# OpenPPL/ppl.llm.serving

Hardware: AMD Instinct MI355X
Metric: decode tokens/sec, LLaMA-7B int8 (W8A16), max-running-batch 1024 (higher is better)
Workload: dtype fp16 activations, int8 weights (W8A16), int8-g8 KV, fp32 accumulate

## Files before the change

### include/pplhip.h

```cpp
#ifndef PPLHIP_H_
#define PPLHIP_H_

#include <stdint.h>
#include <stddef.h>

#ifdef __cplusplus
extern "C" {
#endif

#define PPLHIP_API __attribute__((visibility("default")))

typedef enum pplhip_status {
    PPLHIP_SUCCESS = 0,
    PPLHIP_OTHER_ERROR = -1,
    PPLHIP_INVALID_VALUE = -2,
    PPLHIP_OUT_OF_MEMORY = -3,
    PPLHIP_DEVICE_RUNTIME_ERROR = -4,
    PPLHIP_DEVICE_MEMORY_ERROR = -5,
    PPLHIP_NOT_FOUND = -6,
    PPLHIP_UNSUPPORTED = -7
} pplhip_status;

typedef struct pplhip_model_desc {
    int32_t hidden_dim;
// ... 208 lines not shown
    void* cache;
    void* scale;
    int64_t max_tokens;
    int32_t num_layers;
    int32_t kv_heads;
    int32_t head_dim;
    int32_t quant_bit, quant_group, layout, mode, page_size;
    int32_t layer;
} pplhip_kv_view;

PPLHIP_API int pplhip_op_rope_kv_write(void* stream, void* qkv, const float* cos_sin, const pplhip_kv_view* kv,
                                       const int64_t* seq_starts, const int64_t* start_pos,
                                       const int64_t* cache_indices, int64_t max_pages, int64_t B, int64_t T,
                                       int32_t num_heads);

PPLHIP_API int pplhip_op_attention(void* stream, const void* qkv, const pplhip_kv_view* kv,
                                   const int64_t* seq_starts, const int64_t* start_pos,
                                   const int64_t* cache_indices, int64_t max_pages, int64_t B, int64_t T,
                                   int64_t decoding_batches, int64_t max_seq_len, int64_t max_kv_len,
                                   int32_t num_heads, int32_t split_k, void* workspace, uint64_t workspace_bytes,
                                   void* out);

PPLHIP_API int pplhip_build_rope_table(float* host_out, int32_t max_position, int32_t head_dim, float theta);

#ifdef __cplusplus
}
#endif

#endif
```

### ppl.llm.serving_amd/csrc/k_gemm_dev.h

```cpp
#pragma once
#include "kernels.h"
#include "k_launch.h"

namespace pplhip {

constexpr int G_BN = 128, G_BM = 128, G_BK = 64;

__device__ __forceinline__ int g_swz(int row, int chunk) { return chunk ^ ((row >> 1) & 7); }

enum { EPI_F16 = 0, EPI_F32 = 1, EPI_SWIGLU = 2 };
template <int EPI>
__device__ __forceinline__ void store4(void* yv, int64_t ldy, int64_t m, int n, float v0, float v1, float v2, float v3) {
    if constexpr (EPI == EPI_F32) {
        *reinterpret_cast<float4*>(reinterpret_cast<float*>(yv) + m * ldy + n) = make_float4(v0, v1, v2, v3);
    } else if constexpr (EPI == EPI_F16) {
        const h4 o = {to_h(v0), to_h(v1), to_h(v2), to_h(v3)};
        *reinterpret_cast<uint2*>(reinterpret_cast<uint16_t*>(yv) + m * ldy + n) = __builtin_bit_cast(uint2, o);
    } else {
        const float g0 = round_h(v0), u0 = round_h(v1), g1 = round_h(v2), u1 = round_h(v3);
        const h2 o = {to_h(g0 / (1.0f + __expf(-g0)) * u0), to_h(g1 / (1.0f + __expf(-g1)) * u1)};
        *reinterpret_cast<uint32_t*>(reinterpret_cast<uint16_t*>(yv) + m * ldy + (n >> 1)) = __builtin_bit_cast(uint32_t, o);
    }
}

template <class F>
// ... 288 lines not shown
```

### ppl.llm.serving_amd/csrc/k_gemm_wide.hip

```cpp
#include <stdlib.h>
#include "k_gemm_dev.h"

namespace pplhip {

namespace {

constexpr int WD_BM = 128, WD_NP = 4;
constexpr int WD_XB = WD_BM * G_BK * 2;
constexpr int WD_XP = WD_XB / 1024;

template <int EPI, int ST, int NC, int ABL = 0>
__global__ __launch_bounds__((NC + WD_NP) * 64) void gemm_w8_wide_kernel(const uint16_t* __restrict__ x, const int8_t* __restrict__ w,
                                                                  const uint16_t* __restrict__ scale, int64_t M, int N, int K,
                                                                  void* __restrict__ yv, int64_t ldy, int n_tiles, int m_tiles) {
    constexpr int WD_BN = 32 * NC, WD_NC = NC;
    constexpr int WD_WB = WD_BN * G_BK, WD_WP = WD_WB / 1024;
    constexpr int WD_PP = (WD_XP + WD_WP + WD_NP - 1) / WD_NP;
    extern __shared__ __attribute__((aligned(16))) char smem_wd[];
    char* const Xs0 = smem_wd;
    char* const Wq0 = smem_wd + ST * WD_XB;

    const int id = blockIdx.x;
    const int xcd = id & 7, slot = id >> 3;
    const int nt = xcd + 8 * (slot / m_tiles);
    const int mt = slot % m_tiles;
    if (nt >= n_tiles) return;
    const int n0 = nt * WD_BN;
    const int64_t m0 = (int64_t)mt * WD_BM;

// ... 40 lines not shown
            const int younger = (ktiles - 1 - t) < (D - 1) ? (ktiles - 1 - t) : (D - 1);
            if (younger >= 2) {
                if (npc == WD_PP) asm volatile("s_waitcnt vmcnt(%0)" ::"n"(2 * WD_PP) : "memory");
                else asm volatile("s_waitcnt vmcnt(%0)" ::"n"(2 * WD_PP - 2) : "memory");
            } else if (younger == 1) {
                if (npc == WD_PP) asm volatile("s_waitcnt vmcnt(%0)" ::"n"(WD_PP) : "memory");
                else asm volatile("s_waitcnt vmcnt(%0)" ::"n"(WD_PP - 1) : "memory");
            } else {
                asm volatile("s_waitcnt vmcnt(0)" ::: "memory");
            }
            if (!(ABL & 8)) __syncthreads();
            if (t + D < ktiles && !(ABL & 1)) WD_PRODUCE(t + D, stn);
            stn = stn == ST - 1 ? 0 : stn + 1;
        }
#undef WD_PRODUCE
        return;
    }

    const int l15 = lane & 15, kq = lane >> 4;
    const int nb = wave * 32;
    f4 acc[2][8];
#pragma unroll
    for (int i = 0; i < 2; ++i)
#pragma unroll
        for (int j = 0; j < 8; ++j) acc[i][j] = f4{0.f, 0.f, 0.f, 0.f};
    int st = 0;
    for (int t = 0; t < ktiles; ++t) {
        if (!(ABL & 8)) __syncthreads();
        const uint16_t* xs = reinterpret_cast<const uint16_t*>(Xs0 + st * WD_XB);
        const char* wq = Wq0 + st * WD_WB;
// ... 12 lines not shown
                if constexpr (ABL & 2) a[i] = __builtin_bit_cast(h8, make_uint4(wraw[i].x, wraw[i].y, wraw[i].z ^ ks, wraw[i].w));
                else a[i] = cvt_i8x8_f16(ks == 0 ? make_uint2(wraw[i].x, wraw[i].y) : make_uint2(wraw[i].z, wraw[i].w));
            }
#pragma unroll
            for (int j = 0; j < 8; ++j) {
                const int row = j * 16 + l15;
                bfr[j] = __builtin_bit_cast(h8, *reinterpret_cast<const uint4*>(&xs[((ABL & 4) ? 0 : row * G_BK) + g_swz(row, ks * 4 + kq) * 8]));
            }
#pragma unroll
            for (int i = 0; i < 2; ++i)
#pragma unroll
                for (int j = 0; j < 8; ++j) acc[i][j] = __builtin_amdgcn_mfma_f32_16x16x32_f16(a[i], bfr[j], acc[i][j], 0, 0, 0);
        }
    }

#pragma unroll
    for (int i = 0; i < 2; ++i) {
        const int n = n0 + nb + i * 16 + kq * 4;
        if (n >= N) continue;
        const h4 sh = __builtin_bit_cast(h4, *reinterpret_cast<const uint2*>(scale + n));
#pragma unroll
        for (int j = 0; j < 8; ++j) {
            const int64_t m = m0 + j * 16 + l15;
            if (m >= M) continue;
            store4<EPI>(yv, ldy, m, n, acc[i][j][0] * (float)sh[0], acc[i][j][1] * (float)sh[1], acc[i][j][2] * (float)sh[2],
                        acc[i][j][3] * (float)sh[3]);
        }
    }
}

// ... 15 lines not shown
    const size_t lds = (size_t)ST * (WD_XB + bn * G_BK);
    if (route) {
        route->add("kernel=gemm_w8_wide_kernel<%s,%d,%d> splits=1 reduce=none order=plain", epi_name(epi), ST, nc);
        if (route->dry) return hipSuccess;
    }
    static LdsOptIn once;
    if (once.first()) set_max_lds(lds, gemm_w8_wide_kernel<EPI_F16, ST, 12>, gemm_w8_wide_kernel<EPI_F32, ST, 12>, gemm_w8_wide_kernel<EPI_SWIGLU, ST, 12>);
    dim3 grid((unsigned)((n_tiles + 7) / 8 * 8 * m_tiles));
#ifdef WD_ABLATE_BUILD
    static const int abl = getenv("PPLHIP_GEMM_WIDE_ABLATE") ? atoi(getenv("PPLHIP_GEMM_WIDE_ABLATE")) : 0;
    bool ablated = true;
    dispatch_int<1, 2, 3, 4, 6, 7, 8, 15, 0>(abl, [&](auto A) {
        if constexpr (A == 0) ablated = false;
        else {
            set_max_lds(lds, gemm_w8_wide_kernel<EPI_F16, ST, 12, A>);
            hipLaunchKernelGGL((gemm_w8_wide_kernel<EPI_F16, ST, 12, A>), grid, dim3((12 + WD_NP) * 64), lds, s, x, w, scale, M, N, K, y, ldy, n_tiles, m_tiles);
        }
    });
    if (ablated) return hipGetLastError();
#endif
    dispatch_epi(epi, [&](auto E) {
        hipLaunchKernelGGL((gemm_w8_wide_kernel<E, ST, 12>), grid, dim3((12 + WD_NP) * 64), lds, s, x, w, scale, M, N, K, y, ldy, n_tiles, m_tiles);
    });
    return hipGetLastError();
}

}
```

### ppl.llm.serving_amd/csrc/k_rope_kv.hip

```cpp
#include <stdlib.h>
#include "kernels.h"

namespace pplhip {

template <int QBIT>
__device__ __forceinline__ void store_group8(const KvAddr& kv, int kvsel, int head, int64_t slot, int ch0,
                                             const float* x ) {
    const int64_t base = (int64_t)kvsel * kv.sKV + (int64_t)head * kv.sH + slot * kv.sN + ch0;
    if constexpr (QBIT == 0) {
        *reinterpret_cast<uint4*>(reinterpret_cast<uint16_t*>(kv.cache) + base) = pack8(x);
    } else {
        float mx = 0.f;
#pragma unroll
        for (int i = 0; i < 8; ++i) mx = fmaxf(mx, fabsf(x[i]));
        const _Float16 sh = to_h(mx / 127.0f);
        const float sf = (float)sh;
        const float inv = sf > 0.f ? __fdiv_rn(1.0f, sf) : 0.f;
        uint32_t lo = 0, hi = 0;
#pragma unroll
        for (int i = 0; i < 8; ++i) {
            float q = rintf(__fmul_rn(x[i], inv));
            q = fminf(fmaxf(q, -127.f), 127.f);
            const uint32_t b = (uint32_t)(int)q & 0xffu;
            if (i < 4) lo |= b << (8 * i); else hi |= b << (8 * (i - 4));
        }
        *reinterpret_cast<uint2*>(reinterpret_cast<int8_t*>(kv.cache) + base) = make_uint2(lo, hi);
        const int64_t sbase = (int64_t)kvsel * kv.ssKV + (int64_t)head * kv.ssH + slot * kv.ssN + ch0 / 8;
        kv.scale[sbase] = __builtin_bit_cast(uint16_t, sh);
    }
}

__device__ __forceinline__ void store_fp8_row8(const KvAddr& kv, int kvsel, int head, int64_t slot, int ch0, const float* x ,
                                               int e) {
    const int64_t base = (int64_t)kvsel * kv.sKV + (int64_t)head * kv.sH + slot * kv.sN + ch0;
    const float inv = __builtin_bit_cast(float, (uint32_t)(127 - e) << 23);
    const float lim = e == 8 ? 240.0f : 448.0f;
    uint32_t lo = 0, hi = 0;
#pragma unroll
    for (int i = 0; i < 8; ++i) {
        const float y = __fmul_rn(x[i], inv);
        const uint32_t b = fp8_e4m3_rne(fminf(fmaxf(y, -lim), lim));
        if (i < 4) lo |= b << (8 * i); else hi |= b << (8 * (i - 4));
    }
    *reinterpret_cast<uint2*>(reinterpret_cast<uint8_t*>(kv.cache) + base) = make_uint2(lo, hi);
    if (ch0 == 0) kv.scale[(int64_t)kvsel * kv.ssKV + (int64_t)head * kv.ssH + slot * kv.ssN] = f2h(__builtin_bit_cast(float, (uint32_t)(127 + e) << 23));
}
__device__ __forceinline__ float group_max(float v, int n) {
    for (int o = 1; o < n; o <<= 1) v = fmaxf(v, __shfl_xor(v, o, 64));
    return v;
}

template <int QBIT>
__global__ __launch_bounds__(256) void rope_kv_write_kernel(uint16_t* __restrict__ qkv, const float* __restrict__ cos_sin,
                                                            KvAddr kv, const int64_t* __restrict__ seq_starts,
                                                            const int64_t* __restrict__ start_pos,
                                                            const int64_t* __restrict__ cache_indices, int64_t max_pages,
                                                            int64_t B, int64_t t0, int H, int Hkv, int D, SplitSlabs sl) {
    const int64_t t = t0 + blockIdx.x;
    int64_t b;
    {
        const int64_t g = t < B ? t : B - 1;
        int64_t lo = 0, hi = B - 1;
        if (seq_starts[g] <= t && t < seq_starts[g + 1]) {
            lo = g;
        } else {
            while (lo < hi) {
                const int64_t mid = (lo + hi + 1) >> 1;
                if (seq_starts[mid] <= t) lo = mid; else hi = mid - 1;
            }
        }
        b = lo;
    }
    const int64_t pos = start_pos[b] + (t - seq_starts[b]);
    const int64_t slot = kv_slot(kv, cache_indices, max_pages, b, pos);
    const int half = D / 2;
    const int bph = half / 8;
    const int n_rope = (H + Hkv) * bph;
    const int n_v = Hkv * (D / 8);
    const int v0 = QBIT == KV_FP8 ? (n_rope + D / 8 - 1) / (D / 8) * (D / 8) : n_rope;
    uint16_t* row = qkv + t * (int64_t)(H + 2 * Hkv) * D;
    const float* cs = cos_sin + pos * D;
    for (int w = blockIdx.y * 256 + threadIdx.x; w < v0 + n_v; w += 256 * gridDim.y) {
        if (w < n_rope) {
            const int head = w / bph, i0 = (w - head * bph) * 8;
            uint16_t* x = row + (int64_t)head * D;
            float a[8], bb[8], c[8], s[8], ra[8], rb[8];
            if (sl.splits) {
                slab_load8(sl, t - t0, head * D + i0, a);
                slab_load8(sl, t - t0, head * D + i0 + half, bb);
            } else {
                unpack8(*reinterpret_cast<const uint4*>(x + i0), a);
                unpack8(*reinterpret_cast<const uint4*>(x + i0 + half), bb);
            }
            *reinterpret_cast<float4*>(c) = *reinterpret_cast<const float4*>(cs + i0);
            *reinterpret_cast<float4*>(c + 4) = *reinterpret_cast<const float4*>(cs + i0 + 4);
            *reinterpret_cast<float4*>(s) = *reinterpret_cast<const float4*>(cs + half + i0);
            *reinterpret_cast<float4*>(s + 4) = *reinterpret_cast<const float4*>(cs + half + i0 + 4);
#pragma unroll
            for (int i = 0; i < 8; ++i) {
                ra[i] = round_h(__fsub_rn(__fmul_rn(a[i], c[i]), __fmul_rn(bb[i], s[i])));
                rb[i] = round_h(__fadd_rn(__fmul_rn(bb[i], c[i]), __fmul_rn(a[i], s[i])));
            }
            if (head < H) {
                *reinterpret_cast<uint4*>(x + i0) = pack8(ra);
                *reinterpret_cast<uint4*>(x + i0 + half) = pack8(rb);
            } else if constexpr (QBIT == KV_FP8) {
                float mx = 0.f;
#pragma unroll
                for (int i = 0; i < 8; ++i) mx = fmaxf(mx, fmaxf(fabsf(ra[i]), fabsf(rb[i])));
                const int e = fp8_row_exp(group_max(mx, bph));
                store_fp8_row8(kv, 0, head - H, slot, i0, ra, e);
                store_fp8_row8(kv, 0, head - H, slot, i0 + half, rb, e);
            } else {
                store_group8<QBIT>(kv, 0, head - H, slot, i0, ra);
                store_group8<QBIT>(kv, 0, head - H, slot, i0 + half, rb);
            }
        } else if (w >= v0) {
            const int wv = w - v0;
            const int head = wv / (D / 8), i0 = (wv - head * (D / 8)) * 8;
            float v[8];
            if (sl.splits) slab_load8(sl, t - t0, (H + Hkv + head) * D + i0, v);
            else unpack8(*reinterpret_cast<const uint4*>(row + (int64_t)(H + Hkv + head) * D + i0), v);
            if constexpr (QBIT == KV_FP8) {
                float mx = 0.f;
#pragma unroll
                for (int i = 0; i < 8; ++i) mx = fmaxf(mx, fabsf(v[i]));
                store_fp8_row8(kv, 1, head, slot, i0, v, fp8_row_exp(group_max(mx, D / 8)));
            } else {
                store_group8<QBIT>(kv, 1, head, slot, i0, v);
            }
        }
    }
}

hipError_t launch_rope_kv_write(hipStream_t s, uint16_t* qkv, const float* cos_sin, const KvAddr& kv, int kv_fmt, const int64_t* seq_starts, const int64_t* start_pos,
                                const int64_t* cache_indices, int64_t max_pages, int64_t B, int64_t t0, int64_t T, int H,
                                int Hkv, int D, const SplitSlabs* qkv_slabs) {
    if (T == 0) return hipSuccess;
    SplitSlabs sl;
    if (qkv_slabs && qkv_slabs->splits > 0) {
        sl = *qkv_slabs;
        if (sl.N != (H + 2 * Hkv) * D || sl.M != T) return hipErrorInvalidValue;
    }
    if (D % 16 || (kv_fmt != KV_FP16 && kv_fmt != KV_I8G8 && kv_fmt != KV_FP8)) return hipErrorInvalidValue;
    const int items = (H + Hkv) * (D / 16) + Hkv * (D / 8);
// ... 20 lines not shown
```

### ppl.llm.serving_amd/csrc/kernels.h

```cpp
#pragma once
#include <hip/hip_runtime.h>
#include <stdint.h>
#include "k_common.h"

namespace pplhip {

struct SplitSlabs {
    const float* ws = nullptr;
    int splits = 0;
    const uint16_t* scale = nullptr;
    int N = 0;
    int64_t M = 0;
};
struct LinearRoute {
    char* buf = nullptr;
    int cap = 0;
    int len = 0;
    bool dry = false;
    void add(const char* fmt, ...) __attribute__((format(printf, 2, 3)));
};
inline const char* epi_name(int epi) { return epi == 1 ? "f32" : (epi == 2 ? "swiglu" : "f16"); }
#ifdef __HIPCC__
__device__ __forceinline__ void slab_load8(const SplitSlabs& sl, int64_t m, int n, float* o) {
    const float* p = sl.ws + m * sl.N + n;
// ... 55 lines not shown
                                 const int64_t* start_pos, const int64_t* cache_indices, int64_t max_pages, int64_t b0, int64_t B,
                                 int H, int Hkv, int D, int64_t max_seq_len, uint16_t* out, int64_t max_kv_len = 0, float* ws = nullptr,
                                 size_t ws_bytes = 0, int64_t row0 = 0, int64_t nrows = 0);

bool attn_decode_gqa_supported(int kv_fmt, int H, int Hkv, int D);
hipError_t launch_attn_decode_gqa(hipStream_t s, const uint16_t* qkv, const KvAddr& kv, int kv_fmt,
                                  const int64_t* seq_starts, const int64_t* start_pos, const int64_t* cache_indices,
                                  int64_t max_pages, int64_t nb, int H, int Hkv, int D, int split, float* workspace,
                                  uint16_t* out, hipEvent_t t0 = nullptr, hipEvent_t t1 = nullptr);

hipError_t launch_linear_w8_wide(hipStream_t s, const uint16_t* x, const int8_t* w, const uint16_t* scale, int64_t M, int N, int K, void* y,
                                 int64_t ldy, int epi, int nc, LinearRoute* route = nullptr);
bool linear_w4_pc_supported(int group, int64_t M, int N, int K, const void* x, const void* w, const void* scale, const void* y, int64_t ldy, int epi);
hipError_t launch_linear_w4_pc(hipStream_t s, const uint16_t* x, const void* w, const uint16_t* scale, int64_t M, int N, int K, void* y,
                               int64_t ldy, int epi, LinearRoute* route = nullptr);
int linear_w8_wide_waves(int64_t M, int N);
hipError_t launch_linear(hipStream_t s, const uint16_t* x, const void* w, const uint16_t* scale, int wq_bit, int group,
                         int64_t M, int N, int K, void* y, int64_t ldy, bool out_fp32, float* ws = nullptr, size_t ws_bytes = 0,
                         bool swiglu = false, SplitSlabs* defer = nullptr,
                         LinearRoute* route = nullptr);
hipError_t launch_splitk_reduce(hipStream_t s, const float* ws, int splits, int64_t M, int N, const uint16_t* scale, void* y, int64_t ldy, int epi);
int gemv_stream_max_m(int wq_bit, int group, int N, int K);
hipError_t launch_gemv_stream(hipStream_t s, const uint16_t* x, const void* w, const uint16_t* scale, int wq_bit, int group, int64_t M, int N,
                              int K, void* y, int64_t ldy, int epi, LinearRoute* route = nullptr);
hipError_t launch_quant_act(hipStream_t s, const uint16_t* x, int64_t M, int K, int64_t ldx, int8_t* q, int64_t ldq, float* sx);
hipError_t launch_quant_weight(hipStream_t s, const uint16_t* w, int N, int K, int8_t* q, int64_t ldq, uint16_t* scale);
hipError_t launch_linear_i8(hipStream_t s, const int8_t* xq, const float* sx, const int8_t* w, const uint16_t* scale, int64_t M, int N,
                            int K, void* y, int64_t ldy, bool out_fp32, bool swiglu);
hipError_t launch_quant_act_f8(hipStream_t s, const uint16_t* x, int64_t M, int K, int64_t ldx, uint8_t* q, int64_t ldq, float* sx);
hipError_t launch_quant_weight_f8(hipStream_t s, const uint16_t* w, int N, int K, uint8_t* q, int64_t ldq, uint16_t* scale);
// ... 47 lines not shown
```

### ppl.llm.serving_amd/csrc/pplhip.cc

```cpp
#include "../../include/pplhip.h"

#include <hip/hip_runtime.h>
#include <rccl/rccl.h>

#include <algorithm>
#include <cmath>
#include <cstdio>
#include <cstdlib>
#include <cstring>
#include <map>
#include <unordered_map>
#include <memory>
#include <string>
#include <vector>

#include "kernels.h"

using namespace pplhip;

namespace {

enum { ACT_FP16 = 0, ACT_I8 = 1, ACT_FP8 = 2 };

struct Linear {
// ... 1236 lines not shown
    const pplhip_model_desc& d = c->d;
    hipStream_t s = R.stream;
    const int hd = d.hidden_dim, H = c->H, Hkv = c->Hkv, D = c->D;
    const int nqkv = (H + 2 * Hkv) * D;
    Layer& L = R.layers[l];
    ProfEvent ev;
    uint16_t* h = R.h + k.t0 * hd;
    uint16_t* xn = R.xn + k.t0 * hd;
    const bool a8 = c->act_fmt != ACT_FP16;
    {
        if (!xn_ready)
            HIPCK(c, rank, launch_rmsnorm(s, h, pending ? pending + k.t0 * hd : nullptr, L.attn_norm, d.norm_eps, k.tn, hd, nullptr, xn,
                                          pending ? h : nullptr, a8 ? R.xq : nullptr, a8 ? R.sx : nullptr, pending ? &R.sl_part2 : nullptr,
                                          c->act_fmt == ACT_FP8));
        R.sl_part2 = SplitSlabs{};
        prof_begin(c, R, PPLHIP_PROF_GEMM, &ev);
        { int rc = layer_linear(c, rank, L.wqkv, xn, k.tn, R.qkv + k.t0 * nqkv, L.wqkv.N, false, a8, &R.sl_qkv); if (rc) return rc; }
        prof_end(R, &ev);
    }
    const KvAddr kv = make_kv_addr(d, Hkv, D, R.kv_tokens, R.kv_cache, R.kv_scale, l);
    HIPCK(c, rank, launch_rope_kv_write(s, R.qkv, R.rope, kv, c->kv_fmt, R.d_seq, R.d_sp, R.d_ci,
                                        R.max_pages, R.B, k.t0, k.tn, H, Hkv, D, &R.sl_qkv));
    R.sl_qkv = SplitSlabs{};
    const int64_t ci_stride = d.cache_mode == 1 ? R.max_pages : 1;
    if (k.nd > 0) {
        if (c->o.enable_profiling == 2) {
            std::pair<hipEvent_t, hipEvent_t> p;
            if (!R.prof_free.empty()) { p = R.prof_free.back(); R.prof_free.pop_back(); }
            else { hipEventCreate(&p.first); hipEventCreate(&p.second); }
            ev.cls = PPLHIP_PROF_ATTN_DECODE; ev.a = p.first; ev.b = p.second;
            HIPCK(c, rank, launch_attn_decode(s, R.qkv, kv, c->kv_fmt, R.d_seq + k.b0, R.d_sp + k.b0, R.d_ci + k.b0 * ci_stride,
                                              R.max_pages, k.nd, H, Hkv, D, R.max_kv_len, split, threads, R.attn_ws,
                                              R.att + k.b0 * (int64_t)H * D, ev.a, ev.b));
            R.prof.push_back(ev);
        } else {
            prof_begin(c, R, PPLHIP_PROF_ATTN_DECODE, &ev);
            HIPCK(c, rank, launch_attn_decode(s, R.qkv, kv, c->kv_fmt, R.d_seq + k.b0, R.d_sp + k.b0, R.d_ci + k.b0 * ci_stride,
// ... 666 lines not shown
    d.num_layers = v->num_layers;
    d.cache_quant_bit = v->quant_bit; d.cache_quant_group = v->quant_group;
    d.cache_layout = v->layout; d.cache_mode = v->mode; d.page_size = v->page_size;
    return make_kv_addr(d, v->kv_heads, v->head_dim, (uint64_t)v->max_tokens, v->cache, (uint16_t*)v->scale, v->layer);
}

int pplhip_op_rope_kv_write(void* stream, void* qkv, const float* cos_sin, const pplhip_kv_view* kv, const int64_t* seq_starts,
                            const int64_t* start_pos, const int64_t* cache_indices, int64_t max_pages, int64_t B, int64_t T,
                            int32_t num_heads) {
    const int fmt = kv ? kv_format(kv->quant_bit, kv->quant_group, kv->head_dim) : -1;
    if (fmt < 0) return PPLHIP_INVALID_VALUE;
    return op_rc(launch_rope_kv_write((hipStream_t)stream, (uint16_t*)qkv, cos_sin, view_addr(kv), fmt,
                                      seq_starts, start_pos, cache_indices, max_pages, B, 0, T, num_heads, kv->kv_heads, kv->head_dim));
}

int pplhip_op_attention(void* stream, const void* qkv, const pplhip_kv_view* kv, const int64_t* seq_starts,
                        const int64_t* start_pos, const int64_t* cache_indices, int64_t max_pages, int64_t B, int64_t T,
                        int64_t decoding_batches, int64_t max_seq_len, int64_t max_kv_len, int32_t num_heads, int32_t split_k,
                        void* workspace, uint64_t workspace_bytes, void* out) {
    (void)T;
    const int fmt = kv ? kv_format(kv->quant_bit, kv->quant_group, kv->head_dim) : -1;
    if (fmt < 0) return PPLHIP_INVALID_VALUE;
    const int64_t nb = std::min<int64_t>(std::max<int64_t>(decoding_batches, 0), B);
    int split = split_k < 1 ? 1 : split_k;
    if (split > 1 && attn_decode_workspace_bytes(nb, num_heads, kv->head_dim, split) > workspace_bytes) return PPLHIP_INVALID_VALUE;
    hipStream_t s = (hipStream_t)stream;
    const KvAddr a = view_addr(kv);
    hipError_t e = hipSuccess;
    if (nb > 0)
        e = launch_attn_decode(s, (const uint16_t*)qkv, a, fmt, seq_starts, start_pos, cache_indices, max_pages, nb,
// ... 10 lines not shown
```

### ppl.llm.serving_amd/pplhip.py

```python
import ctypes as C
import os
import struct
import subprocess

import numpy as np

_DIR = os.path.dirname(os.path.abspath(__file__))
LIB_PATH = os.environ.get("PPLHIP_LIB") or os.path.join(_DIR, "csrc", "libpplhip.so")
UNIQUE_ID_BYTES = 128
IPC_HANDLE_BYTES = 64
COMM_NONE, COMM_RCCL, COMM_P2P = 0, 1, 2
_LIB = None

STATUS = {0: "SUCCESS", -1: "OTHER_ERROR", -2: "INVALID_VALUE", -3: "OUT_OF_MEMORY", -4: "DEVICE_RUNTIME_ERROR",
          -5: "DEVICE_MEMORY_ERROR", -6: "NOT_FOUND", -7: "UNSUPPORTED"}

PROF_ATTN_DECODE, PROF_ATTN_PREFILL, PROF_GEMM, PROF_RUN = 0, 1, 2, 3


class PplHipError(RuntimeError):
    pass


class ModelDesc(C.Structure):
# ... 47 lines not shown

class CommInfo(C.Structure):
    _fields_ = [("mode", C.c_int32), ("selftest", C.c_int32), ("schedule", C.c_int32), ("has_rccl", C.c_int32),
                ("dual_min_rows", C.c_int64), ("dual_max_rows", C.c_int64), ("notes", C.c_char * 512)]


SYMBOLS = [
    "pplhip_version", "pplhip_device_count", "pplhip_get_unique_id", "pplhip_init", "pplhip_destroy",
    "pplhip_comm_export", "pplhip_comm_connect", "pplhip_comm_mode", "pplhip_comm_fused_norm", "pplhip_comm_info", "pplhip_comm_allreduce_us",
    "pplhip_last_error", "pplhip_rank_load", "pplhip_rank_set_tensor", "pplhip_rank_init_synthetic", "pplhip_rank_tie_output",
    "pplhip_kv_block_bytes", "pplhip_kv_capacity", "pplhip_kv_alloc", "pplhip_kv_ptrs", "pplhip_kv_read",
    "pplhip_kv_write", "pplhip_kv_fill_synthetic", "pplhip_set_inputs", "pplhip_run", "pplhip_debug_run_dump", "pplhip_logits", "pplhip_copy_logits", "pplhip_sync",
    "pplhip_sample", "pplhip_penalty", "pplhip_profile_reset", "pplhip_profile_get", "pplhip_profile_mode", "pplhip_mem_info",
    "pplhip_op_embedding", "pplhip_op_rmsnorm", "pplhip_op_linear", "pplhip_op_linear_swiglu", "pplhip_op_linear_ex", "pplhip_op_rmsnorm_quant", "pplhip_op_quant_act", "pplhip_op_quant_weight",
    "pplhip_op_linear_i8", "pplhip_op_rmsnorm_quant_f8", "pplhip_op_quant_act_f8", "pplhip_op_quant_weight_f8", "pplhip_op_linear_f8",
    "pplhip_op_silu_mul", "pplhip_op_penalty", "pplhip_op_sample", "pplhip_op_rope_kv_write",
    "pplhip_op_attention", "pplhip_build_rope_table",
]


def build():
    subprocess.check_call(["make", "-s", "-j8", "-C", os.path.join(_DIR, "csrc")])


def lib():
    global _LIB
    if _LIB is None:
        if not os.path.exists(LIB_PATH):
            raise PplHipError(f"{LIB_PATH} is missing: build it with __graft_entry__.build() (no CPU fallback exists)")
        L = C.CDLL(LIB_PATH)
        vp, i32, i64, u64, f32 = C.c_void_p, C.c_int32, C.c_int64, C.c_uint64, C.c_float
# ... 37 lines not shown
        L.pplhip_op_linear.argtypes = [vp, vp, vp, vp, i32, i32, i64, i32, i32, vp, i32]
        L.pplhip_op_linear_swiglu.argtypes = [vp, vp, vp, vp, i32, i32, i64, i32, i32, vp]
        L.pplhip_op_linear_ex.argtypes = [vp, vp, vp, vp, i32, i32, i64, i32, i32, vp, i64, i32, vp, u64, i32, C.c_char_p, i32]
        L.pplhip_op_rmsnorm_quant.argtypes = [vp, vp, vp, vp, C.c_float, i64, i32, vp, vp, vp]
        L.pplhip_op_quant_act.argtypes = [vp, vp, i64, i32, vp, vp]
        L.pplhip_op_quant_weight.argtypes = [vp, vp, i32, i32, vp, vp]
        L.pplhip_op_linear_i8.argtypes = [vp, vp, vp, vp, vp, i64, i32, i32, vp, i32, i32]
        L.pplhip_op_rmsnorm_quant_f8.argtypes = [vp, vp, vp, vp, C.c_float, i64, i32, vp, vp, vp]
        L.pplhip_op_quant_act_f8.argtypes = [vp, vp, i64, i32, vp, vp]
        L.pplhip_op_quant_weight_f8.argtypes = [vp, vp, i32, i32, vp, vp]
        L.pplhip_op_linear_f8.argtypes = [vp, vp, vp, vp, vp, i64, i32, i32, vp, i32, i32]
        L.pplhip_op_silu_mul.argtypes = [vp, vp, i64, i32, vp]
        L.pplhip_op_penalty.argtypes = [vp] * 10 + [i32, i32, i32, i32, vp]
        L.pplhip_op_sample.argtypes = [vp] * 5 + [i32, i32, i32, i32, f32, vp, vp]
        L.pplhip_op_rope_kv_write.argtypes = [vp, vp, vp, C.POINTER(KvView), vp, vp, vp, i64, i64, i64, i32]
        L.pplhip_op_attention.argtypes = [vp, vp, C.POINTER(KvView), vp, vp, vp, i64, i64, i64, i64, i64, i64, i32, i32,
                                          vp, u64, vp]
        L.pplhip_build_rope_table.argtypes = [vp, i32, i32, f32]
        _LIB = L
    return _LIB


def linear_route(x, w, scale, wq_bit, group, M, N, K, y, ldy, epi, ws=None, ws_bytes=0, dry_run=True, stream=None):
    buf = C.create_string_buffer(1024)
    rc = lib().pplhip_op_linear_ex(stream, x, w, scale, wq_bit, group, M, N, K, y, ldy, epi, ws, ws_bytes, int(dry_run), buf, 1024)
    return rc, buf.value.decode()


def make_desc(**kw):
    d = ModelDesc()
    defaults = dict(norm_eps=1e-5, rope_theta=10000.0, max_position=4096, cache_quant_bit=0, cache_quant_group=1,
                    cache_layout=3, cache_mode=0, page_size=0, weight_quant_bit=0, weight_quant_group=128, act_quant_bit=0)
    defaults.update(kw)
    for k, v in defaults.items():
        setattr(d, k, v)
    return d


def copy_desc(src, cls=ModelDesc):
    d = cls()
# ... 259 lines not shown
```

Before: 24110.

## Fuse RoPE and KV-cache write into the wide W8 QKV GEMM epilogue

Adds an EPI_ROPE_KV epilogue to the wide int8-weight GEMM. Each 384-column tile, which holds three heads, stages its scaled fp16 outputs in LDS. The kernel then applies RoPE to Q/K, writes Q back, and quantizes K/V straight into the KV cache, with producer waves looking up each row's position and slot. This removes the separate rope_kv_write launch and its re-read of the QKV buffer for decode batches that qualify for the single-launch wide path. The cost is more epilogue work and barriers inside the GEMM, and a narrower eligibility condition that falls back to the old path otherwise.

```diff
diff --git a/include/pplhip.h b/include/pplhip.h
--- a/include/pplhip.h
+++ b/include/pplhip.h
@@ -246,6 +246,12 @@
                                        const int64_t* cache_indices, int64_t max_pages, int64_t B, int64_t T,
                                        int32_t num_heads);
 
+PPLHIP_API int pplhip_op_linear_rope_kv(void* stream, const void* x, const void* w, const void* scale, int32_t wq_bit, int32_t group,
+                                        int64_t M, int32_t N, int32_t K, void* qkv, const float* cos_sin, const pplhip_kv_view* kv,
+                                        const int64_t* seq_starts, const int64_t* start_pos, const int64_t* cache_indices,
+                                        int64_t max_pages, int64_t B, int64_t T, int32_t num_heads, int32_t deferred_splits,
+                                        int32_t dry_run, char* route, int32_t route_len);
+
 PPLHIP_API int pplhip_op_attention(void* stream, const void* qkv, const pplhip_kv_view* kv,
                                    const int64_t* seq_starts, const int64_t* start_pos,
                                    const int64_t* cache_indices, int64_t max_pages, int64_t B, int64_t T,
diff --git a/ppl.llm.serving_amd/csrc/k_gemm_dev.h b/ppl.llm.serving_amd/csrc/k_gemm_dev.h
--- a/ppl.llm.serving_amd/csrc/k_gemm_dev.h
+++ b/ppl.llm.serving_amd/csrc/k_gemm_dev.h
@@ -8,7 +8,7 @@
 
 __device__ __forceinline__ int g_swz(int row, int chunk) { return chunk ^ ((row >> 1) & 7); }
 
-enum { EPI_F16 = 0, EPI_F32 = 1, EPI_SWIGLU = 2 };
+enum { EPI_F16 = 0, EPI_F32 = 1, EPI_SWIGLU = 2, EPI_ROPE_KV = 3 };
 template <int EPI>
 __device__ __forceinline__ void store4(void* yv, int64_t ldy, int64_t m, int n, float v0, float v1, float v2, float v3) {
     if constexpr (EPI == EPI_F32) {
diff --git a/ppl.llm.serving_amd/csrc/k_gemm_wide.hip b/ppl.llm.serving_amd/csrc/k_gemm_wide.hip
--- a/ppl.llm.serving_amd/csrc/k_gemm_wide.hip
+++ b/ppl.llm.serving_amd/csrc/k_gemm_wide.hip
@@ -1,5 +1,6 @@
 #include <stdlib.h>
 #include "k_gemm_dev.h"
+#include "k_rope_kv_dev.h"
 
 namespace pplhip {
 
@@ -9,10 +10,41 @@
 constexpr int WD_XB = WD_BM * G_BK * 2;
 constexpr int WD_XP = WD_XB / 1024;
 
-template <int EPI, int ST, int NC, int ABL = 0>
+constexpr int WD_RK_LD = 384 * 2 + 16;
+constexpr int WD_RK_ROWINFO = WD_BM * WD_RK_LD;
+
+template <int QB>
+__device__ __forceinline__ void wide_rope_kv_items(char* smem, int tid, int first_lookup_tid, int64_t m0, int64_t M, int n0, uint16_t* y, int64_t ldy,
+                                                   const RopeKvArgs& rk) {
+    constexpr int D = 128;
+    int64_t* rowinfo = reinterpret_cast<int64_t*>(smem + WD_RK_ROWINFO);
+    {
+        const int r = tid - first_lookup_tid;
+        if (r >= 0 && r < WD_BM && m0 + r < M)
+            rope_kv_row_lookup(rk.kv, rk.seq_starts, rk.start_pos, rk.cache_indices, rk.max_pages, rk.B, rk.t0 + m0 + r, &rowinfo[2 * r], &rowinfo[2 * r + 1]);
+    }
+    __syncthreads();
+    const int r = tid >> 3, g = tid & 7;
+    const int64_t m = m0 + r;
+    if (m >= M) return;
+    const int64_t pos = rowinfo[2 * r], slot = rowinfo[2 * r + 1];
+    const char* trow = smem + r * WD_RK_LD;
+    auto load8 = [&](int n, float* o) { unpack8(*reinterpret_cast<const uint4*>(trow + (n - n0) * 2), o); };
+    const int heads = rk.H + 2 * rk.Hkv;
+#pragma unroll 1
+    for (int h = 0; h < 3; ++h) {
+        const int head = n0 / D + h;
+        if (head >= heads) break;
+        if (head < rk.H + rk.Hkv) rope_kv_rope_item<QB>(load8, head, g * 8, rk.H, D, y + m * ldy, rk.cos_sin + pos * D, rk.kv, slot, 8);
+        else rope_kv_v_item<QB, 2>(load8, head - rk.H - rk.Hkv, g * 8, rk.H, rk.Hkv, D, rk.kv, slot, 8);
+    }
+}
+
+template <int EPI, int ST, int NC, int ABL = 0, int QB = 0>
 __global__ __launch_bounds__((NC + WD_NP) * 64) void gemm_w8_wide_kernel(const uint16_t* __restrict__ x, const int8_t* __restrict__ w,
                                                                   const uint16_t* __restrict__ scale, int64_t M, int N, int K,
-                                                                  void* __restrict__ yv, int64_t ldy, int n_tiles, int m_tiles) {
+                                                                  void* __restrict__ yv, int64_t ldy, int n_tiles, int m_tiles, RopeKvArgs rk) {
+    static_assert(EPI != EPI_ROPE_KV || (NC == 12 && ST * (WD_XB + 32 * NC * G_BK) >= WD_RK_ROWINFO + WD_BM * 16), "EPI_ROPE_KV: three heads per tile, staged in the ring");
     constexpr int WD_BN = 32 * NC, WD_NC = NC;
     constexpr int WD_WB = WD_BN * G_BK, WD_WP = WD_WB / 1024;
     constexpr int WD_PP = (WD_XP + WD_WP + WD_NP - 1) / WD_NP;
@@ -83,6 +115,10 @@
             stn = stn == ST - 1 ? 0 : stn + 1;
         }
 #undef WD_PRODUCE
+        if constexpr (EPI == EPI_ROPE_KV) {
+            __syncthreads();
+            wide_rope_kv_items<QB>(smem_wd, tid, WD_NC * 64, m0, M, n0, reinterpret_cast<uint16_t*>(yv), ldy, rk);
+        }
         return;
     }
 
@@ -125,6 +161,23 @@
         }
     }
 
+    if constexpr (EPI == EPI_ROPE_KV) {
+        __syncthreads();
+#pragma unroll
+        for (int i = 0; i < 2; ++i) {
+            const int nl = nb + i * 16 + kq * 4;
+            if (n0 + nl >= N) continue;
+            const h4 sh = __builtin_bit_cast(h4, *reinterpret_cast<const uint2*>(scale + n0 + nl));
+#pragma unroll
+            for (int j = 0; j < 8; ++j) {
+                const h4 o = {to_h(acc[i][j][0] * (float)sh[0]), to_h(acc[i][j][1] * (float)sh[1]), to_h(acc[i][j][2] * (float)sh[2]),
+                              to_h(acc[i][j][3] * (float)sh[3])};
+                *reinterpret_cast<uint2*>(smem_wd + (j * 16 + l15) * WD_RK_LD + nl * 2) = __builtin_bit_cast(uint2, o);
+            }
+        }
+        wide_rope_kv_items<QB>(smem_wd, tid, WD_NC * 64, m0, M, n0, reinterpret_cast<uint16_t*>(yv), ldy, rk);
+        return;
+    }
 #pragma unroll
     for (int i = 0; i < 2; ++i) {
         const int n = n0 + nb + i * 16 + kq * 4;
@@ -170,15 +223,53 @@
         if constexpr (A == 0) ablated = false;
         else {
             set_max_lds(lds, gemm_w8_wide_kernel<EPI_F16, ST, 12, A>);
-            hipLaunchKernelGGL((gemm_w8_wide_kernel<EPI_F16, ST, 12, A>), grid, dim3((12 + WD_NP) * 64), lds, s, x, w, scale, M, N, K, y, ldy, n_tiles, m_tiles);
+            hipLaunchKernelGGL((gemm_w8_wide_kernel<EPI_F16, ST, 12, A>), grid, dim3((12 + WD_NP) * 64), lds, s, x, w, scale, M, N, K, y, ldy, n_tiles, m_tiles, RopeKvArgs{});
         }
     });
     if (ablated) return hipGetLastError();
 #endif
     dispatch_epi(epi, [&](auto E) {
-        hipLaunchKernelGGL((gemm_w8_wide_kernel<E, ST, 12>), grid, dim3((12 + WD_NP) * 64), lds, s, x, w, scale, M, N, K, y, ldy, n_tiles, m_tiles);
+        hipLaunchKernelGGL((gemm_w8_wide_kernel<E, ST, 12>), grid, dim3((12 + WD_NP) * 64), lds, s, x, w, scale, M, N, K, y, ldy, n_tiles, m_tiles, RopeKvArgs{});
     });
     return hipGetLastError();
 }
 
-}
+bool linear_w8_wide_single_launch(int64_t M, int N, int K) {
+    if (tune_int("PPLHIP_GEMM_WIDE", 1) != 1 || tune_set("PPLHIP_GEMM_GENERIC")) return false;
+    const int msplit = tune_int("PPLHIP_GEMM_MSPLIT", 256);
+    if (msplit && M > 1024 && M < 3584 && (M & 1023) != 0 && (M & 1023) <= msplit) return false;
+    return K % G_BK == 0 && M >= 512 && M < 4096 && N >= 8192 && linear_w8_wide_waves(M, N) == 12;
+}
+
+hipError_t launch_linear_w8_wide_rope_kv(hipStream_t s, const uint16_t* x, const int8_t* w, const uint16_t* scale, int64_t M, int N, int K,
+                                         uint16_t* qkv, const float* cos_sin, const KvAddr& kv, int kv_fmt, const int64_t* seq_starts,
+                                         const int64_t* start_pos, const int64_t* cache_indices, int64_t max_pages, int64_t B, int64_t t0, int H,
+                                         int Hkv, int D, const SplitSlabs* qkv_slabs, LinearRoute* route) {
+    if (D != 128 || (qkv_slabs && qkv_slabs->splits > 0)) return hipErrorInvalidValue;
+    if (H <= 0 || Hkv <= 0 || N != (H + 2 * Hkv) * D || K <= 0 || K % G_BK) return hipErrorInvalidValue;
+    if (kv_fmt != KV_FP16 && kv_fmt != KV_I8G8 && kv_fmt != KV_FP8) return hipErrorInvalidValue;
+    if (M == 0) return hipSuccess;
+    constexpr int ST = 3, NC = 12;
+    const int n_tiles = (N + 32 * NC - 1) / (32 * NC), m_tiles = (int)((M + WD_BM - 1) / WD_BM);
+    const size_t lds = (size_t)ST * (WD_XB + 32 * NC * G_BK);
+    if (route) {
+        route->add("kernel=gemm_w8_wide_kernel<rope_kv,%d,%d> splits=1 reduce=none order=plain rope_kv=fused kv=%s", ST, NC,
+                   kv_fmt == KV_I8G8 ? "i8g8" : (kv_fmt == KV_FP8 ? "fp8" : "fp16"));
+        if (route->dry) return hipSuccess;
+    }
+    static LdsOptIn once;
+    if (once.first())
+        set_max_lds(lds, gemm_w8_wide_kernel<EPI_ROPE_KV, ST, NC, 0, KV_FP16>, gemm_w8_wide_kernel<EPI_ROPE_KV, ST, NC, 0, KV_I8G8>,
+                    gemm_w8_wide_kernel<EPI_ROPE_KV, ST, NC, 0, KV_FP8>);
+    RopeKvArgs rk;
+    rk.cos_sin = cos_sin; rk.kv = kv; rk.seq_starts = seq_starts; rk.start_pos = start_pos; rk.cache_indices = cache_indices;
+    rk.max_pages = max_pages; rk.B = B; rk.t0 = t0; rk.H = H; rk.Hkv = Hkv;
+    dim3 grid((unsigned)((n_tiles + 7) / 8 * 8 * m_tiles));
+    dispatch_int<KV_I8G8, KV_FP8, KV_FP16>(kv_fmt, [&](auto Q) {
+        hipLaunchKernelGGL((gemm_w8_wide_kernel<EPI_ROPE_KV, ST, NC, 0, Q>), grid, dim3((NC + WD_NP) * 64), lds, s, x, w, scale, M, N, K,
+                           (void*)(qkv + t0 * (int64_t)N), (int64_t)N, n_tiles, m_tiles, rk);
+    });
+    return hipGetLastError();
+}
+
+}
diff --git a/ppl.llm.serving_amd/csrc/k_rope_kv.hip b/ppl.llm.serving_amd/csrc/k_rope_kv.hip
--- a/ppl.llm.serving_amd/csrc/k_rope_kv.hip
+++ b/ppl.llm.serving_amd/csrc/k_rope_kv.hip
@@ -1,54 +1,7 @@
 #include <stdlib.h>
-#include "kernels.h"
+#include "k_rope_kv_dev.h"
 
 namespace pplhip {
-
-template <int QBIT>
-__device__ __forceinline__ void store_group8(const KvAddr& kv, int kvsel, int head, int64_t slot, int ch0,
-                                             const float* x ) {
-    const int64_t base = (int64_t)kvsel * kv.sKV + (int64_t)head * kv.sH + slot * kv.sN + ch0;
-    if constexpr (QBIT == 0) {
-        *reinterpret_cast<uint4*>(reinterpret_cast<uint16_t*>(kv.cache) + base) = pack8(x);
-    } else {
-        float mx = 0.f;
-#pragma unroll
-        for (int i = 0; i < 8; ++i) mx = fmaxf(mx, fabsf(x[i]));
-        const _Float16 sh = to_h(mx / 127.0f);
-        const float sf = (float)sh;
-        const float inv = sf > 0.f ? __fdiv_rn(1.0f, sf) : 0.f;
-        uint32_t lo = 0, hi = 0;
-#pragma unroll
-        for (int i = 0; i < 8; ++i) {
-            float q = rintf(__fmul_rn(x[i], inv));
-            q = fminf(fmaxf(q, -127.f), 127.f);
-            const uint32_t b = (uint32_t)(int)q & 0xffu;
-            if (i < 4) lo |= b << (8 * i); else hi |= b << (8 * (i - 4));
-        }
-        *reinterpret_cast<uint2*>(reinterpret_cast<int8_t*>(kv.cache) + base) = make_uint2(lo, hi);
-        const int64_t sbase = (int64_t)kvsel * kv.ssKV + (int64_t)head * kv.ssH + slot * kv.ssN + ch0 / 8;
-        kv.scale[sbase] = __builtin_bit_cast(uint16_t, sh);
-    }
-}
-
-__device__ __forceinline__ void store_fp8_row8(const KvAddr& kv, int kvsel, int head, int64_t slot, int ch0, const float* x ,
-                                               int e) {
-    const int64_t base = (int64_t)kvsel * kv.sKV + (int64_t)head * kv.sH + slot * kv.sN + ch0;
-    const float inv = __builtin_bit_cast(float, (uint32_t)(127 - e) << 23);
-    const float lim = e == 8 ? 240.0f : 448.0f;
-    uint32_t lo = 0, hi = 0;
-#pragma unroll
-    for (int i = 0; i < 8; ++i) {
-        const float y = __fmul_rn(x[i], inv);
-        const uint32_t b = fp8_e4m3_rne(fminf(fmaxf(y, -lim), lim));
-        if (i < 4) lo |= b << (8 * i); else hi |= b << (8 * (i - 4));
-    }
-    *reinterpret_cast<uint2*>(reinterpret_cast<uint8_t*>(kv.cache) + base) = make_uint2(lo, hi);
-    if (ch0 == 0) kv.scale[(int64_t)kvsel * kv.ssKV + (int64_t)head * kv.ssH + slot * kv.ssN] = f2h(__builtin_bit_cast(float, (uint32_t)(127 + e) << 23));
-}
-__device__ __forceinline__ float group_max(float v, int n) {
-    for (int o = 1; o < n; o <<= 1) v = fmaxf(v, __shfl_xor(v, o, 64));
-    return v;
-}
 
 template <int QBIT>
 __global__ __launch_bounds__(256) void rope_kv_write_kernel(uint16_t* __restrict__ qkv, const float* __restrict__ cos_sin,
@@ -57,22 +10,8 @@
                                                             const int64_t* __restrict__ cache_indices, int64_t max_pages,
                                                             int64_t B, int64_t t0, int H, int Hkv, int D, SplitSlabs sl) {
     const int64_t t = t0 + blockIdx.x;
-    int64_t b;
-    {
-        const int64_t g = t < B ? t : B - 1;
-        int64_t lo = 0, hi = B - 1;
-        if (seq_starts[g] <= t && t < seq_starts[g + 1]) {
-            lo = g;
-        } else {
-            while (lo < hi) {
-                const int64_t mid = (lo + hi + 1) >> 1;
-                if (seq_starts[mid] <= t) lo = mid; else hi = mid - 1;
-            }
-        }
-        b = lo;
-    }
-    const int64_t pos = start_pos[b] + (t - seq_starts[b]);
-    const int64_t slot = kv_slot(kv, cache_indices, max_pages, b, pos);
+    int64_t pos, slot;
+    rope_kv_row_lookup(kv, seq_starts, start_pos, cache_indices, max_pages, B, t, &pos, &slot);
     const int half = D / 2;
     const int bph = half / 8;
     const int n_rope = (H + Hkv) * bph;
@@ -80,55 +19,18 @@
     const int v0 = QBIT == KV_FP8 ? (n_rope + D / 8 - 1) / (D / 8) * (D / 8) : n_rope;
     uint16_t* row = qkv + t * (int64_t)(H + 2 * Hkv) * D;
     const float* cs = cos_sin + pos * D;
+    auto load8 = [&](int n, float* o) {
+        if (sl.splits) slab_load8(sl, t - t0, n, o);
+        else unpack8(*reinterpret_cast<const uint4*>(row + n), o);
+    };
     for (int w = blockIdx.y * 256 + threadIdx.x; w < v0 + n_v; w += 256 * gridDim.y) {
         if (w < n_rope) {
             const int head = w / bph, i0 = (w - head * bph) * 8;
-            uint16_t* x = row + (int64_t)head * D;
-            float a[8], bb[8], c[8], s[8], ra[8], rb[8];
-            if (sl.splits) {
-                slab_load8(sl, t - t0, head * D + i0, a);
-                slab_load8(sl, t - t0, head * D + i0 + half, bb);
-            } else {
-                unpack8(*reinterpret_cast<const uint4*>(x + i0), a);
-                unpack8(*reinterpret_cast<const uint4*>(x + i0 + half), bb);
-            }
-            *reinterpret_cast<float4*>(c) = *reinterpret_cast<const float4*>(cs + i0);
-            *reinterpret_cast<float4*>(c + 4) = *reinterpret_cast<const float4*>(cs + i0 + 4);
-            *reinterpret_cast<float4*>(s) = *reinterpret_cast<const float4*>(cs + half + i0);
-            *reinterpret_cast<float4*>(s + 4) = *reinterpret_cast<const float4*>(cs + half + i0 + 4);
-#pragma unroll
-            for (int i = 0; i < 8; ++i) {
-                ra[i] = round_h(__fsub_rn(__fmul_rn(a[i], c[i]), __fmul_rn(bb[i], s[i])));
-                rb[i] = round_h(__fadd_rn(__fmul_rn(bb[i], c[i]), __fmul_rn(a[i], s[i])));
-            }
-            if (head < H) {
-                *reinterpret_cast<uint4*>(x + i0) = pack8(ra);
-                *reinterpret_cast<uint4*>(x + i0 + half) = pack8(rb);
-            } else if constexpr (QBIT == KV_FP8) {
-                float mx = 0.f;
-#pragma unroll
-                for (int i = 0; i < 8; ++i) mx = fmaxf(mx, fmaxf(fabsf(ra[i]), fabsf(rb[i])));
-                const int e = fp8_row_exp(group_max(mx, bph));
-                store_fp8_row8(kv, 0, head - H, slot, i0, ra, e);
-                store_fp8_row8(kv, 0, head - H, slot, i0 + half, rb, e);
-            } else {
-                store_group8<QBIT>(kv, 0, head - H, slot, i0, ra);
-                store_group8<QBIT>(kv, 0, head - H, slot, i0 + half, rb);
-            }
+            rope_kv_rope_item<QBIT>(load8, head, i0, H, D, row, cs, kv, slot, bph);
         } else if (w >= v0) {
             const int wv = w - v0;
             const int head = wv / (D / 8), i0 = (wv - head * (D / 8)) * 8;
-            float v[8];
-            if (sl.splits) slab_load8(sl, t - t0, (H + Hkv + head) * D + i0, v);
-            else unpack8(*reinterpret_cast<const uint4*>(row + (int64_t)(H + Hkv + head) * D + i0), v);
-            if constexpr (QBIT == KV_FP8) {
-                float mx = 0.f;
-#pragma unroll
-                for (int i = 0; i < 8; ++i) mx = fmaxf(mx, fabsf(v[i]));
-                store_fp8_row8(kv, 1, head, slot, i0, v, fp8_row_exp(group_max(mx, D / 8)));
-            } else {
-                store_group8<QBIT>(kv, 1, head, slot, i0, v);
-            }
+            rope_kv_v_item<QBIT, 1>(load8, head, i0, H, Hkv, D, kv, slot, D / 8);
         }
     }
 }
diff --git a/ppl.llm.serving_amd/csrc/k_rope_kv_dev.h b/ppl.llm.serving_amd/csrc/k_rope_kv_dev.h
--- /dev/null
+++ b/ppl.llm.serving_amd/csrc/k_rope_kv_dev.h
@@ -0,0 +1,134 @@
+#pragma once
+#include "kernels.h"
+
+namespace pplhip {
+
+template <int QBIT>
+__device__ __forceinline__ void store_group8(const KvAddr& kv, int kvsel, int head, int64_t slot, int ch0,
+                                             const float* x ) {
+    const int64_t base = (int64_t)kvsel * kv.sKV + (int64_t)head * kv.sH + slot * kv.sN + ch0;
+    if constexpr (QBIT == 0) {
+        *reinterpret_cast<uint4*>(reinterpret_cast<uint16_t*>(kv.cache) + base) = pack8(x);
+    } else {
+        float mx = 0.f;
+#pragma unroll
+        for (int i = 0; i < 8; ++i) mx = fmaxf(mx, fabsf(x[i]));
+        const _Float16 sh = to_h(mx / 127.0f);
+        const float sf = (float)sh;
+        const float inv = sf > 0.f ? __fdiv_rn(1.0f, sf) : 0.f;
+        uint32_t lo = 0, hi = 0;
+#pragma unroll
+        for (int i = 0; i < 8; ++i) {
+            float q = rintf(__fmul_rn(x[i], inv));
+            q = fminf(fmaxf(q, -127.f), 127.f);
+            const uint32_t b = (uint32_t)(int)q & 0xffu;
+            if (i < 4) lo |= b << (8 * i); else hi |= b << (8 * (i - 4));
+        }
+        *reinterpret_cast<uint2*>(reinterpret_cast<int8_t*>(kv.cache) + base) = make_uint2(lo, hi);
+        const int64_t sbase = (int64_t)kvsel * kv.ssKV + (int64_t)head * kv.ssH + slot * kv.ssN + ch0 / 8;
+        kv.scale[sbase] = __builtin_bit_cast(uint16_t, sh);
+    }
+}
+
+__device__ __forceinline__ void store_fp8_row8(const KvAddr& kv, int kvsel, int head, int64_t slot, int ch0, const float* x ,
+                                               int e) {
+    const int64_t base = (int64_t)kvsel * kv.sKV + (int64_t)head * kv.sH + slot * kv.sN + ch0;
+    const float inv = __builtin_bit_cast(float, (uint32_t)(127 - e) << 23);
+    const float lim = e == 8 ? 240.0f : 448.0f;
+    uint32_t lo = 0, hi = 0;
+#pragma unroll
+    for (int i = 0; i < 8; ++i) {
+        const float y = __fmul_rn(x[i], inv);
+        const uint32_t b = fp8_e4m3_rne(fminf(fmaxf(y, -lim), lim));
+        if (i < 4) lo |= b << (8 * i); else hi |= b << (8 * (i - 4));
+    }
+    *reinterpret_cast<uint2*>(reinterpret_cast<uint8_t*>(kv.cache) + base) = make_uint2(lo, hi);
+    if (ch0 == 0) kv.scale[(int64_t)kvsel * kv.ssKV + (int64_t)head * kv.ssH + slot * kv.ssN] = f2h(__builtin_bit_cast(float, (uint32_t)(127 + e) << 23));
+}
+__device__ __forceinline__ float group_max(float v, int n) {
+    for (int o = 1; o < n; o <<= 1) v = fmaxf(v, __shfl_xor(v, o, 64));
+    return v;
+}
+__device__ __forceinline__ float absmax8(const float* x ) {
+    float mx = 0.f;
+#pragma unroll
+    for (int i = 0; i < 8; ++i) mx = fmaxf(mx, fabsf(x[i]));
+    return mx;
+}
+
+__device__ __forceinline__ void rope_kv_row_lookup(const KvAddr& kv, const int64_t* __restrict__ seq_starts, const int64_t* __restrict__ start_pos,
+                                                   const int64_t* __restrict__ cache_indices, int64_t max_pages, int64_t B, int64_t t,
+                                                   int64_t* pos_out, int64_t* slot_out) {
+    int64_t b;
+    {
+        const int64_t g = t < B ? t : B - 1;
+        int64_t lo = 0, hi = B - 1;
+        if (seq_starts[g] <= t && t < seq_starts[g + 1]) {
+            lo = g;
+        } else {
+            while (lo < hi) {
+                const int64_t mid = (lo + hi + 1) >> 1;
+                if (seq_starts[mid] <= t) lo = mid; else hi = mid - 1;
+            }
+        }
+        b = lo;
+    }
+    const int64_t pos = start_pos[b] + (t - seq_starts[b]);
+    *pos_out = pos;
+    *slot_out = kv_slot(kv, cache_indices, max_pages, b, pos);
+}
+
+__device__ __forceinline__ void rope_rotate8(const float* a, const float* bb, const float* __restrict__ cs, int i0, int half, float* ra, float* rb) {
+    float c[8], s[8];
+    *reinterpret_cast<float4*>(c) = *reinterpret_cast<const float4*>(cs + i0);
+    *reinterpret_cast<float4*>(c + 4) = *reinterpret_cast<const float4*>(cs + i0 + 4);
+    *reinterpret_cast<float4*>(s) = *reinterpret_cast<const float4*>(cs + half + i0);
+    *reinterpret_cast<float4*>(s + 4) = *reinterpret_cast<const float4*>(cs + half + i0 + 4);
+#pragma unroll
+    for (int i = 0; i < 8; ++i) {
+        ra[i] = round_h(__fsub_rn(__fmul_rn(a[i], c[i]), __fmul_rn(bb[i], s[i])));
+        rb[i] = round_h(__fadd_rn(__fmul_rn(bb[i], c[i]), __fmul_rn(a[i], s[i])));
+    }
+}
+
+template <int QBIT, class Load8>
+__device__ __forceinline__ void rope_kv_rope_item(Load8&& load8, int head, int i0, int H, int D, uint16_t* qrow,
+                                                  const float* __restrict__ cs, const KvAddr& kv, int64_t slot, int fp8_lanes) {
+    const int half = D / 2;
+    float a[8], bb[8], ra[8], rb[8];
+    load8(head * D + i0, a);
+    load8(head * D + i0 + half, bb);
+    rope_rotate8(a, bb, cs, i0, half, ra, rb);
+    if (head < H) {
+        uint16_t* x = qrow + (int64_t)head * D;
+        *reinterpret_cast<uint4*>(x + i0) = pack8(ra);
+        *reinterpret_cast<uint4*>(x + i0 + half) = pack8(rb);
+    } else if constexpr (QBIT == KV_FP8) {
+        const int e = fp8_row_exp(group_max(fmaxf(absmax8(ra), absmax8(rb)), fp8_lanes));
+        store_fp8_row8(kv, 0, head - H, slot, i0, ra, e);
+        store_fp8_row8(kv, 0, head - H, slot, i0 + half, rb, e);
+    } else {
+        store_group8<QBIT>(kv, 0, head - H, slot, i0, ra);
+        store_group8<QBIT>(kv, 0, head - H, slot, i0 + half, rb);
+    }
+}
+
+template <int QBIT, int NG, class Load8>
+__device__ __forceinline__ void rope_kv_v_item(Load8&& load8, int head, int i0, int H, int Hkv, int D, const KvAddr& kv, int64_t slot,
+                                               int fp8_lanes) {
+    float v[NG][8];
+#pragma unroll
+    for (int g = 0; g < NG; ++g) load8((H + Hkv + head) * D + i0 + g * (D / 2), v[g]);
+    if constexpr (QBIT == KV_FP8) {
+        float mx = absmax8(v[0]);
+        if constexpr (NG == 2) mx = fmaxf(mx, absmax8(v[1]));
+        const int e = fp8_row_exp(group_max(mx, fp8_lanes));
+#pragma unroll
+        for (int g = 0; g < NG; ++g) store_fp8_row8(kv, 1, head, slot, i0 + g * (D / 2), v[g], e);
+    } else {
+#pragma unroll
+        for (int g = 0; g < NG; ++g) store_group8<QBIT>(kv, 1, head, slot, i0 + g * (D / 2), v[g]);
+    }
+}
+
+}
diff --git a/ppl.llm.serving_amd/csrc/kernels.h b/ppl.llm.serving_amd/csrc/kernels.h
--- a/ppl.llm.serving_amd/csrc/kernels.h
+++ b/ppl.llm.serving_amd/csrc/kernels.h
@@ -93,6 +93,20 @@
 bool linear_w4_pc_supported(int group, int64_t M, int N, int K, const void* x, const void* w, const void* scale, const void* y, int64_t ldy, int epi);
 hipError_t launch_linear_w4_pc(hipStream_t s, const uint16_t* x, const void* w, const uint16_t* scale, int64_t M, int N, int K, void* y,
                                int64_t ldy, int epi, LinearRoute* route = nullptr);
+struct RopeKvArgs {
+    const float* cos_sin = nullptr;
+    KvAddr kv = {};
+    const int64_t* seq_starts = nullptr;
+    const int64_t* start_pos = nullptr;
+    const int64_t* cache_indices = nullptr;
+    int64_t max_pages = 0, B = 0, t0 = 0;
+    int H = 0, Hkv = 0;
+};
+hipError_t launch_linear_w8_wide_rope_kv(hipStream_t s, const uint16_t* x, const int8_t* w, const uint16_t* scale, int64_t M, int N, int K,
+                                         uint16_t* qkv, const float* cos_sin, const KvAddr& kv, int kv_fmt, const int64_t* seq_starts,
+                                         const int64_t* start_pos, const int64_t* cache_indices, int64_t max_pages, int64_t B, int64_t t0, int H,
+                                         int Hkv, int D, const SplitSlabs* qkv_slabs = nullptr, LinearRoute* route = nullptr);
+bool linear_w8_wide_single_launch(int64_t M, int N, int K);
 int linear_w8_wide_waves(int64_t M, int N);
 hipError_t launch_linear(hipStream_t s, const uint16_t* x, const void* w, const uint16_t* scale, int wq_bit, int group,
                          int64_t M, int N, int K, void* y, int64_t ldy, bool out_fp32, float* ws = nullptr, size_t ws_bytes = 0,
diff --git a/ppl.llm.serving_amd/csrc/pplhip.cc b/ppl.llm.serving_amd/csrc/pplhip.cc
--- a/ppl.llm.serving_amd/csrc/pplhip.cc
+++ b/ppl.llm.serving_amd/csrc/pplhip.cc
@@ -1274,13 +1274,22 @@
                                           pending ? h : nullptr, a8 ? R.xq : nullptr, a8 ? R.sx : nullptr, pending ? &R.sl_part2 : nullptr,
                                           c->act_fmt == ACT_FP8));
         R.sl_part2 = SplitSlabs{};
+    }
+    const KvAddr kv = make_kv_addr(d, Hkv, D, R.kv_tokens, R.kv_cache, R.kv_scale, l);
+    static const bool fuse_rope = tune_int("PPLHIP_QKV_ROPE_FUSE", 1) != 0;
+    const Linear& wq = L.wqkv;
+    if (fuse_rope && !a8 && wq.qbit == 8 && D == 128 && wq.N == nqkv && linear_w8_wide_single_launch(k.tn, wq.N, wq.Kp)) {
         prof_begin(c, R, PPLHIP_PROF_GEMM, &ev);
-        { int rc = layer_linear(c, rank, L.wqkv, xn, k.tn, R.qkv + k.t0 * nqkv, L.wqkv.N, false, a8, &R.sl_qkv); if (rc) return rc; }
+        HIPCK(c, rank, launch_linear_w8_wide_rope_kv(s, xn, (const int8_t*)wq.w, wq.scale, k.tn, wq.N, wq.Kp, R.qkv, R.rope, kv, c->kv_fmt, R.d_seq,
+                                                     R.d_sp, R.d_ci, R.max_pages, R.B, k.t0, H, Hkv, D));
         prof_end(R, &ev);
-    }
-    const KvAddr kv = make_kv_addr(d, Hkv, D, R.kv_tokens, R.kv_cache, R.kv_scale, l);
-    HIPCK(c, rank, launch_rope_kv_write(s, R.qkv, R.rope, kv, c->kv_fmt, R.d_seq, R.d_sp, R.d_ci,
-                                        R.max_pages, R.B, k.t0, k.tn, H, Hkv, D, &R.sl_qkv));
+    } else {
+        prof_begin(c, R, PPLHIP_PROF_GEMM, &ev);
+        { int rc = layer_linear(c, rank, wq, xn, k.tn, R.qkv + k.t0 * nqkv, wq.N, false, a8, &R.sl_qkv); if (rc) return rc; }
+        prof_end(R, &ev);
+        HIPCK(c, rank, launch_rope_kv_write(s, R.qkv, R.rope, kv, c->kv_fmt, R.d_seq, R.d_sp, R.d_ci,
+                                            R.max_pages, R.B, k.t0, k.tn, H, Hkv, D, &R.sl_qkv));
+    }
     R.sl_qkv = SplitSlabs{};
     const int64_t ci_stride = d.cache_mode == 1 ? R.max_pages : 1;
     if (k.nd > 0) {
@@ -1977,6 +1986,25 @@
                                       seq_starts, start_pos, cache_indices, max_pages, B, 0, T, num_heads, kv->kv_heads, kv->head_dim));
 }
 
+int pplhip_op_linear_rope_kv(void* stream, const void* x, const void* w, const void* scale, int32_t wq_bit, int32_t group, int64_t M, int32_t N,
+                             int32_t K, void* qkv, const float* cos_sin, const pplhip_kv_view* kv, const int64_t* seq_starts,
+                             const int64_t* start_pos, const int64_t* cache_indices, int64_t max_pages, int64_t B, int64_t T, int32_t num_heads,
+                             int32_t deferred_splits, int32_t dry_run, char* route, int32_t route_len) {
+    (void)group;
+    LinearRoute r;
+    r.buf = route_len > 0 ? route : nullptr;
+    r.cap = route_len;
+    r.dry = dry_run != 0;
+    if (r.buf) r.buf[0] = 0;
+    const int fmt = kv ? kv_format(kv->quant_bit, kv->quant_group, kv->head_dim) : -1;
+    if (fmt < 0 || wq_bit != 8 || T != M || deferred_splits < 0) return PPLHIP_INVALID_VALUE;
+    SplitSlabs sl;
+    sl.splits = deferred_splits;
+    return op_rc(launch_linear_w8_wide_rope_kv((hipStream_t)stream, (const uint16_t*)x, (const int8_t*)w, (const uint16_t*)scale, M, N, K,
+                                               (uint16_t*)qkv, cos_sin, view_addr(kv), fmt, seq_starts, start_pos, cache_indices, max_pages, B, 0,
+                                               num_heads, kv->kv_heads, kv->head_dim, &sl, &r));
+}
+
 int pplhip_op_attention(void* stream, const void* qkv, const pplhip_kv_view* kv, const int64_t* seq_starts,
                         const int64_t* start_pos, const int64_t* cache_indices, int64_t max_pages, int64_t B, int64_t T,
                         int64_t decoding_batches, int64_t max_seq_len, int64_t max_kv_len, int32_t num_heads, int32_t split_k,
diff --git a/ppl.llm.serving_amd/pplhip.py b/ppl.llm.serving_amd/pplhip.py
--- a/ppl.llm.serving_amd/pplhip.py
+++ b/ppl.llm.serving_amd/pplhip.py
@@ -85,7 +85,7 @@
     "pplhip_sample", "pplhip_penalty", "pplhip_profile_reset", "pplhip_profile_get", "pplhip_profile_mode", "pplhip_mem_info",
     "pplhip_op_embedding", "pplhip_op_rmsnorm", "pplhip_op_linear", "pplhip_op_linear_swiglu", "pplhip_op_linear_ex", "pplhip_op_rmsnorm_quant", "pplhip_op_quant_act", "pplhip_op_quant_weight",
     "pplhip_op_linear_i8", "pplhip_op_rmsnorm_quant_f8", "pplhip_op_quant_act_f8", "pplhip_op_quant_weight_f8", "pplhip_op_linear_f8",
-    "pplhip_op_silu_mul", "pplhip_op_penalty", "pplhip_op_sample", "pplhip_op_rope_kv_write",
+    "pplhip_op_silu_mul", "pplhip_op_penalty", "pplhip_op_sample", "pplhip_op_rope_kv_write", "pplhip_op_linear_rope_kv",
     "pplhip_op_attention", "pplhip_build_rope_table",
 ]
 
@@ -153,6 +153,8 @@
         L.pplhip_op_penalty.argtypes = [vp] * 10 + [i32, i32, i32, i32, vp]
         L.pplhip_op_sample.argtypes = [vp] * 5 + [i32, i32, i32, i32, f32, vp, vp]
         L.pplhip_op_rope_kv_write.argtypes = [vp, vp, vp, C.POINTER(KvView), vp, vp, vp, i64, i64, i64, i32]
+        L.pplhip_op_linear_rope_kv.argtypes = [vp, vp, vp, vp, i32, i32, i64, i32, i32, vp, vp, C.POINTER(KvView), vp, vp, vp, i64, i64, i64, i32,
+                                               i32, i32, C.c_char_p, i32]
         L.pplhip_op_attention.argtypes = [vp, vp, C.POINTER(KvView), vp, vp, vp, i64, i64, i64, i64, i64, i64, i32, i32,
                                           vp, u64, vp]
         L.pplhip_build_rope_table.argtypes = [vp, i32, i32, f32]
@@ -163,6 +165,14 @@
 def linear_route(x, w, scale, wq_bit, group, M, N, K, y, ldy, epi, ws=None, ws_bytes=0, dry_run=True, stream=None):
     buf = C.create_string_buffer(1024)
     rc = lib().pplhip_op_linear_ex(stream, x, w, scale, wq_bit, group, M, N, K, y, ldy, epi, ws, ws_bytes, int(dry_run), buf, 1024)
+    return rc, buf.value.decode()
+
+
+def linear_rope_kv(x, w, scale, M, N, K, qkv, cos_sin, view, seq_starts, start_pos, cache_indices, max_pages, B, num_heads,
+                   deferred_splits=0, dry_run=False, stream=None):
+    buf = C.create_string_buffer(1024)
+    rc = lib().pplhip_op_linear_rope_kv(stream, x, w, scale, 8, 0, M, N, K, qkv, cos_sin, C.byref(view), seq_starts, start_pos, cache_indices,
+                                        max_pages, B, M, num_heads, deferred_splits, int(dry_run), buf, 1024)
     return rc, buf.value.decode()
 
 
```

Measured after the change: 24400 (median of 2 runs). No clear change (+1.2%).
